# CaptainEven/DenseBox

Hardware: AMD Instinct MI355X
Metric: training patches/sec (240x240) (higher is better)
Workload: dtype f16; 1 GPU; full training step (fwd + fused dense loss w/ hard-negative mining + bwd + grad all-reduce + SGD) of DenseBoxLMLOC on 240x240 patches; net=DenseBoxLMLOC, batch_per_gpu=64, global_batch=64, patch=240x240, parallelism=dp1, half_neg=11, grad_finite=True

## Files before the change

densebox_amd/_lib.py:

```python
import ctypes as C
import os

_HERE = os.path.dirname(os.path.abspath(__file__))
LIB_PATH = os.environ.get('DBX_LIB') or os.path.join(_HERE, 'csrc', 'libdensebox_hip.so')

F16, BF16, F32 = 0, 1, 2
DTYPE_ID = {'f16': F16, 'bf16': BF16, 'f32': F32}
ESIZE = {F16: 2, BF16: 2, F32: 4}

EPI_BIAS, EPI_RELU, EPI_GATE, EPI_DROPMASK, EPI_ACCUM, EPI_F32_NCHW, EPI_DROPHASH = 1, 2, 4, 8, 16, 32, 64
CONV_WFRAG = 128
K_IGEMM, K_DMA, K_BAND, K_C64, K_C8, K_WS, K_P8 = 1, 2, 3, 4, 5, 6, 7


class View(C.Structure):
    _fields_ = [('ptr', C.c_void_p), ('n', C.c_int32), ('h', C.c_int32), ('w', C.c_int32),
                ('pad', C.c_int32), ('ld', C.c_int32), ('c_off', C.c_int32), ('c', C.c_int32)]


class ConvDesc(C.Structure):
    _fields_ = [('dtype', C.c_int32), ('kh', C.c_int32), ('kw', C.c_int32), ('cpad', C.c_int32),
                ('cin_pad', C.c_int32), ('cout_pad', C.c_int32), ('epilogue', C.c_int32), ('drop_seed', C.c_uint32)]


# ... 168 lines not shown
    'dbx_patch_plan_host': (C.c_int, [_I32, _I32, _I32, _VP, _I32, _D, _D, _D, _I32, C.POINTER(PatchGeom)]),
    'dbx_patch_draw': (C.c_int, [_I64, _I64, _I32, _I32, _VP]),
    'dbx_patch_check_tables': (C.c_int, [_VP, _I32, _VP, _I32, _VP, _I32]),
    'dbx_patch_aug_plan': (C.c_int, [C.POINTER(PatchAugIO), C.POINTER(PatchAugCfg), _I32, _VP]),
    'dbx_patch_augment': (C.c_int, [_VP, _VP, _VP, _VP, _I32, _I32, _I32, _VP, _VP]),
    'dbx_patch_aug_params_host': (C.c_int, [C.POINTER(PatchAugCfg), _I64, _I64, _VP, _VP, _I32, _VP, _VP, _VP, _VP, _VP]),
    'dbx_patch_augment_host': (C.c_int, [_VP, _VP, _VP, _I32, _I32, _VP]),
    'dbx_conv_wgrad_scratch_bytes': (_I64, [_I32, _PV, _PV, _I32, _I32]),
    'dbx_conv_wgrad': (C.c_int, [_I32, _PV, _PV, _I32, _I32, _I32, _I32, _I32, _VP, _VP, _VP, _I32, _VP]),
    'dbx_conv_wgrad_slice': (C.c_int, [_I32, _PV, _PV, _I32, _I32, _I32, _I32, _I32, _VP, _I32, _I32, _VP, _VP, _I32, _VP]),
    'dbx_conv_wgrad_pool_dz_ok': (C.c_int, [_I32, _PV, _PV, _I32, _I32]),
    'dbx_conv_wgrad_pool_dz': (C.c_int, [_I32, _PV, _VP, _I32, _PV, _PV, _I32, _I32, _I32, _I32, _I32, _VP, _VP, _VP, _I32, _I32, _VP]),
    'dbx_head2_backward_up_fused': (C.c_int, [_I32, _PV, _PV]),
    'dbx_heads1_wgrad_gen_ok': (C.c_int, [_I32, _PV, _I32]),
    'dbx_heads1_dgrad_gen': (C.c_int, [_I32, _PV, C.POINTER(C.c_void_p), C.POINTER(C.c_int32), _I32, _I32, C.c_uint32, _VP, _PV, _PV, _VP]),
    'dbx_heads1_wgrad_gen': (C.c_int, [_I32, _PV, _PV, C.POINTER(C.c_void_p), C.POINTER(C.c_int32), _I32, _I32, C.c_uint32, _I32, _VP, _I32, _I32,
                             _VP, _VP, _VP]),
    'dbx_conv_wgrad_plan': (C.c_int, [_I32, _PV, _PV, _I32, _I32, C.c_char_p, _I32, C.POINTER(C.c_int32)]),
    'dbx_nchw_to_framed': (C.c_int, [_I32, _VP, _I32, _PV, _VP]),
    'dbx_u8hwc_to_framed': (C.c_int, [_I32, _VP, _PV, C.POINTER(C.c_float), C.POINTER(C.c_float), _VP]),
    'dbx_nchw_to_framed_ch': (C.c_int, [_I32, _VP, _I32, _PV, _I32, _VP]),
    'dbx_nchw_to_framed_slots': (C.c_int, [_I32, _VP, _VP, _I32, _I32, _PV, _VP]),
    'dbx_framed_to_nchw_f32': (C.c_int, [_I32, _PV, _VP, _VP]),
    'dbx_framed_add_ch': (C.c_int, [_I32, _PV, _I32, _I32, _PV, _I32, _VP]),
    'dbx_maxpool2x2': (C.c_int, [_I32, _PV, _PV, _VP]),
    'dbx_maxpool2x2_bwd': (C.c_int, [_I32, _PV, _PV, _PV, _I32, _I32, _VP]),
    'dbx_maxpool_idx_bytes': (C.c_int64, [_I32, _I32, _I32, _I32]),
    'dbx_maxpool2x2_idx': (C.c_int, [_I32, _PV, _PV, _VP, _VP]),
    'dbx_maxpool2x2_bwd_idx': (C.c_int, [_I32, _VP, _PV, _PV, _I32, _I32, _VP]),
    'dbx_upsample_bilinear': (C.c_int, [_I32, _PV, _PV, _VP]),
    'dbx_upsample_bilinear_bwd': (C.c_int, [_I32, _PV, _PV, _PV, _VP]),
    'dbx_loss_scratch_bytes': (C.c_int64, [_I32]),
    'dbx_loss_forward_backward': (C.c_int, [C.POINTER(LossDesc), C.POINTER(LossIO), _VP, _VP]),
    'dbx_count_positives': (C.c_int, [_VP, _VP, _I32, _VP, _VP]),
    'dbx_init_score_map': (C.c_int, [_VP, _VP, _I32, _VP, _VP]),
    'dbx_init_offset_map': (C.c_int, [_VP, _VP, _I32, _I32, _VP, _VP]),
    'dbx_init_lm_heatmap': (C.c_int, [_VP, _VP, _I32, _I32, _VP, _VP]),
# ... 65 lines not shown
```

densebox_amd/csrc/aux_ops.hip:

```cpp
#include "common.hpp"
#include <mutex>

static thread_local char g_err[512] = "";
void dbx_set_error(const char* fmt, ...) {
    va_list ap;
    va_start(ap, fmt);
    vsnprintf(g_err, sizeof(g_err), fmt, ap);
    va_end(ap);
}
extern "C" const char* dbx_last_error(void) { return g_err; }
extern "C" int dbx_version(void) { return DBX_ABI_VERSION; }
extern "C" int dbx_device_arch(int device) {
    hipDeviceProp_t p;
    if (hipGetDeviceProperties(&p, device) != hipSuccess) { dbx_set_error("hipGetDeviceProperties failed"); return DBX_ERR_HIP; }
    int arch = 0;
    const char* s = p.gcnArchName;
    if (s[0] == 'g' && s[1] == 'f' && s[2] == 'x') arch = (int)strtol(s + 3, nullptr, 16) == 0x950 ? 950 : (int)strtol(s + 3, nullptr, 10);
    return arch;
}

template <typename T> struct Vec { static constexpr int N = 16 / sizeof(T); };

template <typename T> __device__ __forceinline__ void load_vec(const T* p, float (&v)[16 / sizeof(T)]) {
    const u32x4 raw = *(const u32x4*)p;
// ... 38 lines not shown
    }
}
template <typename T> static int nchw_to_framed_t(const float* x, int csrc, const dbx_view* y, hipStream_t s) {
    VIEW_VEC_CHECK(T, y, "nchw_to_framed");
    FrameGeo g = make_geo<T>(y);
    const int64_t total = (int64_t)y->n * y->h * y->w * (y->c / Vec<T>::N);
    hipLaunchKernelGGL(nchw_to_framed_kernel<T>, dim3(grid_for(total)), dim3(256), 0, s, x, csrc, g);
    DBX_LAUNCH_CHECK();
    return DBX_OK;
}
extern "C" int dbx_nchw_to_framed(int32_t dtype, const float* x_nchw, int32_t c_src, const dbx_view* y, void* stream) {
    DBX_DISPATCH_DTYPE(dtype, nchw_to_framed_t, x_nchw, c_src, y, (hipStream_t)stream);
}

struct SlotSrc { const float* x[4]; int k[4]; };
template <typename T>
__global__ void nchw_to_framed_slots_kernel(SlotSrc src, int nslots, int slot, FrameGeo y) {
    constexpr int V = Vec<T>::N;
    const int gps = slot / V, cg = nslots * gps;
    const int64_t total = (int64_t)y.n * y.h * y.w * cg;
    for (int64_t i = blockIdx.x * (int64_t)blockDim.x + threadIdx.x; i < total; i += (int64_t)gridDim.x * blockDim.x) {
        const int px = (int)(i % y.w);
        const int g = (int)((i / y.w) % cg);
        const int py = (int)((i / ((int64_t)y.w * cg)) % y.h);
        const int n = (int)(i / ((int64_t)y.w * cg * y.h));
        const int si = g / gps, c0 = (g % gps) * V;
        const float* x = si == 0 ? src.x[0] : si == 1 ? src.x[1] : si == 2 ? src.x[2] : src.x[3];
        const int k = si == 0 ? src.k[0] : si == 1 ? src.k[1] : si == 2 ? src.k[2] : src.k[3];
        float v[V];
#pragma unroll
        for (int j = 0; j < V; ++j) {
            const int c = c0 + j;
            v[j] = (x && c < k) ? x[(((int64_t)n * k + c) * y.h + py) * y.w + px] : 0.f;
        }
        store_vec<T>((T*)y.base + geo_pix(y, n, py, px) + si * slot + c0, v);
    }
}
template <typename T> static int nchw_to_framed_slots_t(const float* const* xs, const int32_t* ks, int nslots, int slot, const dbx_view* y, hipStream_t s) {
    VIEW_VEC_CHECK(T, y, "nchw_to_framed_slots");
    DBX_REQUIRE(nslots >= 1 && nslots <= 4 && slot % Vec<T>::N == 0 && y->c == nslots * slot, "nchw_to_framed_slots: 1..4 slots of a multiple of the vector width, view of nslots * slot channels");
    SlotSrc src;
    for (int i = 0; i < 4; ++i) {
        src.x[i] = i < nslots ? xs[i] : nullptr; src.k[i] = i < nslots ? ks[i] : 0;
        if (i < nslots) DBX_REQUIRE(ks[i] >= 0 && ks[i] <= slot, "nchw_to_framed_slots: k must fit its slot");
    }
    FrameGeo g = make_geo<T>(y);
    const int64_t total = (int64_t)y->n * y->h * y->w * (y->c / Vec<T>::N);
    hipLaunchKernelGGL(nchw_to_framed_slots_kernel<T>, dim3(grid_for(total)), dim3(256), 0, s, src, nslots, slot, g);
    DBX_LAUNCH_CHECK();
    return DBX_OK;
}
extern "C" int dbx_nchw_to_framed_slots(int32_t dtype, const float* const* x_nchw, const int32_t* k, int32_t nslots, int32_t slot, const dbx_view* y,
                                        void* stream) {
    if (!x_nchw || !k || !y) { dbx_set_error("nchw_to_framed_slots: null argument"); return DBX_ERR_ARG; }
    DBX_DISPATCH_DTYPE(dtype, nchw_to_framed_slots_t, x_nchw, k, nslots, slot, y, (hipStream_t)stream);
}

template <typename T>
__global__ void framed_to_nchw_kernel(FrameGeo x, float* __restrict__ y) {
    const int64_t total = (int64_t)x.n * x.c * x.h * x.w;
    for (int64_t i = blockIdx.x * (int64_t)blockDim.x + threadIdx.x; i < total; i += (int64_t)gridDim.x * blockDim.x) {
        const int px = (int)(i % x.w);
        const int py = (int)((i / x.w) % x.h);
        const int c = (int)((i / ((int64_t)x.w * x.h)) % x.c);
        const int n = (int)(i / ((int64_t)x.w * x.h * x.c));
        y[i] = to_f32(((const T*)x.base)[geo_pix(x, n, py, px) + c]);
    }
}
template <typename T> static int framed_to_nchw_t(const dbx_view* x, float* y, hipStream_t s) {
    FrameGeo g = make_geo<T>(x);
// ... 1708 lines not shown
```

densebox_amd/csrc/conv_igemm.hip:

```cpp
#include "common.hpp"
#include <vector>
#include <stdlib.h>
#include <string.h>

struct ConvArgs {
    const char* x;
    const char* w;
    const float* bias;
    char* y;
    const char* gate;
    const unsigned char* dropmask;
    int M, HoWo, Wo;
    int x_hp, x_wp, x_ld, x_org;
    int y_hp, y_wp, y_ld, y_pad;
    int g_hp, g_wp, g_ld, g_pad;
    int kw;
    int ntaps;
    int cpt;
    int ksteps;
    int ktot_bytes;
    int cout_valid;
    int ntile_n;
    int nblocks;
    int epi;
// ... 1841 lines not shown
    DBX_LAUNCH_CHECK();
    return DBX_OK;
}

extern "C" int dbx_pack_weight(int32_t dtype, int32_t mode, const float* w_oihw, int32_t co, int32_t ci, int32_t kh,
                               int32_t kw, void* w_packed, int32_t rows_pad, int32_t cin_pad, int32_t row_off,
                               int32_t k_off, void* stream) {
    DBX_DISPATCH_DTYPE(dtype, pack_weight_t, mode, w_oihw, co, ci, kh, kw, w_packed, rows_pad, cin_pad, row_off, k_off,
                       (hipStream_t)stream);
}

int dbx_internal_heads1_dgrad_gen_f32(const dbx_view* d_out, const float* const* w2, const int32_t* k, int nh, int use_hash, unsigned seed,
                                      const void* w1t_plain, const dbx_view* y, const dbx_view* gate, hipStream_t s);
template <typename T>
static int heads1_dgrad_gen_t(const dbx_view* d_out, const float* const* w2, const int32_t* k, int nh, int use_hash, unsigned seed, const void* w1t_frag,
                              const dbx_view* y, const dbx_view* gate, hipStream_t s) {
    if constexpr (sizeof(T) != 2) return dbx_internal_heads1_dgrad_gen_f32(d_out, w2, k, nh, use_hash, seed, w1t_frag, y, gate, s);
    else {
        DBX_REQUIRE(nh >= 1 && nh <= 4 && d_out->pad == 0 && d_out->n == y->n && d_out->h == y->h && d_out->w == y->w && gate->n == y->n &&
                    gate->h == y->h && gate->w == y->w, "heads1_dgrad_gen: d_out (compact), y and gate are maps of the same pixels");
        DBX_REQUIRE(y->c == 256 && gate->c == 256 && (y->ld * 2) % 16 == 0 && (gate->ld * 2) % 16 == 0 && (y->c_off * 2) % 16 == 0 && (gate->c_off * 2) % 16 == 0 &&
                    ((size_t)y->ptr % 16) == 0 && ((size_t)gate->ptr % 16) == 0 && ((size_t)w1t_frag % 16) == 0, "heads1_dgrad_gen: 256 output channels, 16-byte aligned");
        DBX_REQUIRE(d_out->c % nh == 0 && d_out->c / nh >= 8 && ((size_t)d_out->ptr % 16) == 0 && (d_out->ld * 2) % 16 == 0 && (d_out->c_off * 2) % 16 == 0 &&
                    ((d_out->c / nh) * 2) % 16 == 0, "heads1_dgrad_gen: d_out slots of >= 8 channels, 16-byte aligned");
        const int64_t npix = (int64_t)y->n * y->h * y->w;
        DBX_REQUIRE(npix > 0 && npix < (1 << 24) && npix * d_out->ld * 2 < ((int64_t)1 << 32), "heads1_dgrad_gen: pixel count");
        HGenArgs a;
        a.g.dout = (const char*)d_out->ptr + (size_t)d_out->c_off * 2;
        for (int i = 0; i < 4; ++i) {
            a.g.w2[i] = i < nh ? w2[i] : nullptr; a.g.k[i] = i < nh ? k[i] : 0;
            if (i < nh) DBX_REQUIRE(w2[i] && k[i] >= 1 && k[i] <= 8, "heads1_dgrad_gen: k in 1..8");
        }
        a.g.ld = d_out->ld; a.g.slot = d_out->c / nh; a.g.nh = nh; a.g.H = y->h; a.g.W = y->w; a.g.pad = 0; a.g.seed = seed; a.g.use_hash = use_hash ? 1 : 0;
        a.w1f = (const char*)w1t_frag;
        a.y = (char*)y->ptr + (size_t)y->c_off * 2; a.gate = (const char*)gate->ptr + (size_t)gate->c_off * 2;
        a.y_hp = y->h + 2 * y->pad; a.y_wp = y->w + 2 * y->pad; a.y_ld = y->ld; a.y_pad = y->pad;
        a.g_hp = gate->h + 2 * gate->pad; a.g_wp = gate->w + 2 * gate->pad; a.g_ld = gate->ld; a.g_pad = gate->pad;
        a.npix = (int)npix; a.ntiles = (int)((npix + 255) / 256); a.nhb = 16 * nh;
        return launch_heads1_dgrad_gen<T>(a, s);
    }
}
extern "C" int dbx_heads1_dgrad_gen(int32_t dtype, const dbx_view* d_out, const float* const* w2, const int32_t* k, int32_t nh, int32_t use_hash,
                                    uint32_t drop_seed, const void* w1t_frag, const dbx_view* y, const dbx_view* gate, void* stream) {
    if (!d_out || !w2 || !k || !w1t_frag || !y || !gate) { dbx_set_error("heads1_dgrad_gen: null argument"); return DBX_ERR_ARG; }
    DBX_DISPATCH_DTYPE(dtype, heads1_dgrad_gen_t, d_out, w2, k, nh, use_hash, (unsigned)drop_seed, w1t_frag, y, gate, (hipStream_t)stream);
}
```

densebox_amd/csrc/heads_gen.hpp:

```cpp
#pragma once

#ifndef HG_ABL
#define HG_ABL 0
#endif
namespace hgen {
constexpr int HB_BYTES = 16384, NST = 4, W2T_BYTES = 2048 * 16 + 64, LUT_BYTES = 256 * 16;
constexpr int SMEM = NST * HB_BYTES + W2T_BYTES + LUT_BYTES;
}
struct HGenArgs {
    GenHid g;
    const char* w1f;
    char* y; const char* gate;
    int y_hp, y_wp, y_ld, y_pad, g_hp, g_wp, g_ld, g_pad;
    int npix, ntiles, nhb;
};

template <typename T>
__global__ __launch_bounds__(256, 1) void heads1_dgrad_gen_kernel(const HGenArgs a) {
    static_assert(sizeof(T) == 2, "16-bit compute types");
    using namespace hgen;
    extern __shared__ __attribute__((aligned(16))) char smem[];
    char* const w2t = smem + NST * HB_BYTES;
    char* const lut = w2t + W2T_BYTES;
    const int tid = threadIdx.x, lane = tid & 63, l31 = lane & 31, lh = lane >> 5;
    const int wave = __builtin_amdgcn_readfirstlane(tid >> 6);
    const int nhb = a.nhb;
    {
        const float sc = a.g.use_hash ? 2.f : 1.f;
        for (int c = tid; c < 32 * nhb; c += 256) {
            const int hd = c >> 9, cl = c & 511;
// ... 30 lines not shown
        unsigned keep;
        asm volatile("s_mov_b32 %0, m0\n\ts_mov_b32 m0, %3\n\ts_nop 0\n\tglobal_load_lds_dwordx4 %1, %2\n\ts_mov_b32 m0, %0"
                     : "=&s"(keep) : "v"(voff), "s"(src), "s"(dst) : "memory");
    };
    const unsigned vlane = (unsigned)lane * 16u;
    int wb_next = 0, st_next = 0;
    auto issue = [&]() {
        const char* src = a.w1f + (size_t)wb_next * HB_BYTES + wave * 4096;
        const unsigned dst = lds0 + st_next * HB_BYTES + wave * 4096;
#pragma unroll
        for (int q = 0; q < 4; ++q) glds(src + q * 1024, vlane, dst + q * 1024);
        if (++wb_next == nhb) wb_next = 0;
        st_next = (st_next + 1) & 3;
    };

    const int stride = gridDim.x;
    int tile = blockIdx.x;
    if (tile >= a.ntiles) return;
    int m[2]; unsigned hm[2]; bool ok[2];
    auto set_tile = [&](int t) {
#pragma unroll
        for (int pf = 0; pf < 2; ++pf) {
            const int mm = t * 256 + wave * 64 + pf * 32 + l31;
            ok[pf] = mm < a.npix;
            m[pf] = ok[pf] ? mm : a.npix - 1;
            hm[pf] = (unsigned)m[pf] * 0x9E3779B1u;
        }
    };
    u32x4 dnx[2];
    auto dfetch = [&](int t, int hd) {
// ... 46 lines not shown
                for (int p = 0; p < 4; ++p)
                    o[p] = __builtin_bit_cast(unsigned, __builtin_convertvector((f32x2v){dd[pf][8 * t + 2 * p], dd[pf][8 * t + 2 * p + 1]}, t2v)) & mk[pf][t][p];
                bfr[buf][pf][t] = o;
            }
    };
    auto gen = [&](int buf, int hb, const u32x4& wa) { gen_mma(wa); gen_masks(hb); gen_pack(buf); };

    f32x16 acc[2][8];
#pragma unroll
    for (int pf = 0; pf < 2; ++pf)
#pragma unroll
        for (int cf = 0; cf < 8; ++cf)
#pragma unroll
            for (int r = 0; r < 16; ++r) acc[pf][cf][r] = 0.f;

    issue(); issue(); issue();
    set_tile(tile);
    dfetch(tile, 0);
    asm volatile("s_waitcnt vmcnt(0)" : "+v"(dnx[0]), "+v"(dnx[1]) :: "memory");
    __syncthreads();
    dswap();
    gen(0, 0, gen_w(0));

    int st = 0;
    for (;;) {
        for (int hb = 0; hb < nhb; hb += 2) {
#pragma unroll
            for (int par = 0; par < 2; ++par) {
                const int h = hb + par;
                asm volatile("s_waitcnt vmcnt(8)" : "+v"(dnx[0]), "+v"(dnx[1]) :: "memory");
                __builtin_amdgcn_s_barrier();
                const char* S = smem + st * HB_BYTES + lane * 16;
                const bool last = h + 1 == nhb;
                const u32x4 wa = gen_w(last ? 0 : h + 1);
                u32x4 wf0[8], wf1[8];
#pragma unroll
                for (int cf = 0; cf < 8; ++cf) wf0[cf] = *(const u32x4*)(S + cf * 1024);
                __builtin_amdgcn_sched_barrier(0);
                if (!(HG_ABL & 8)) issue();
                if ((h & 15) == 12) {
                    const bool wrap = h + 4 >= nhb;
                    dfetch(wrap ? tile + stride : tile, wrap ? 0 : (h + 4) >> 4);
                }
                if ((h & 15) == 15) {
                    if (last) set_tile(tile + stride);
                    dswap();
                }
                if (!(HG_ABL & 1)) { gen_mma(wa); gen_masks(last ? 0 : h + 1); }
                __builtin_amdgcn_sched_barrier(0);
#pragma unroll
                for (int cf = 0; cf < 8; ++cf) {
                    wf1[cf] = *(const u32x4*)(S + (8 + cf) * 1024);
                    if (HG_ABL & 4) continue;
                    Mma32<T>::run(wf0[cf], bfr[par][0][0], acc[0][cf]);
                    Mma32<T>::run(wf0[cf], bfr[par][1][0], acc[1][cf]);
                    __builtin_amdgcn_sched_group_barrier(0x100, 1, 0);
                    __builtin_amdgcn_sched_group_barrier(0x008, 2, 0);
                }
                __builtin_amdgcn_sched_barrier(0);
                if (!(HG_ABL & 1)) gen_pack(par ^ 1);
#pragma unroll
                for (int cf = 0; cf < 8; ++cf) {
                    if (HG_ABL & 4) continue;
                    Mma32<T>::run(wf1[cf], bfr[par][0][1], acc[0][cf]);
                    Mma32<T>::run(wf1[cf], bfr[par][1][1], acc[1][cf]);
                    __builtin_amdgcn_sched_group_barrier(0x008, 2, 0);
                    __builtin_amdgcn_sched_group_barrier(0x002, 4, 0);
                }
                st = (st + 1) & 3;
            }
        }
        __builtin_amdgcn_sched_barrier(0);
        if (!(HG_ABL & 2)) {
            T* ypix[2];
            bool okp[2];
            u32x4 gt[2][8][2];
#pragma unroll
            for (int pf = 0; pf < 2; ++pf) {
                const int mm = tile * 256 + wave * 64 + pf * 32 + l31;
                okp[pf] = mm < a.npix;
                const int mc = okp[pf] ? mm : 0;
                const int hw = a.g.H * a.g.W;
                const int n = mc / hw, rem = mc - n * hw, oy = rem / a.g.W, ox = rem - oy * a.g.W;
                ypix[pf] = (T*)a.y + (size_t)((n * a.y_hp + oy + a.y_pad) * a.y_wp + ox + a.y_pad) * (size_t)a.y_ld + 8 * lh;
                const T* gpix = (const T*)a.gate + (size_t)((n * a.g_hp + oy + a.g_pad) * a.g_wp + ox + a.g_pad) * (size_t)a.g_ld + 8 * lh;
#pragma unroll
                for (int cf = 0; cf < 8; ++cf)
// ... 13 lines not shown
                            T p4[4] = {from_f32<T>(acc[pf][cf][4 * j]), from_f32<T>(acc[pf][cf][4 * j + 1]), from_f32<T>(acc[pf][cf][4 * j + 2]),
                                       from_f32<T>(acc[pf][cf][4 * j + 3])};
                            pk[jj] = *(const u32x2*)p4;
                        }
                        const auto r0 = __builtin_amdgcn_permlane32_swap(pk[0].x, pk[1].x, false, false);
                        const auto r1 = __builtin_amdgcn_permlane32_swap(pk[0].y, pk[1].y, false, false);
                        const u32x4 o = gate_packed16((u32x4){r0[0], r1[0], r0[1], r1[1]}, gt[pf][cf][jp]);
                        if (okp[pf]) *(u32x4*)(ypix[pf] + cf * 32 + 16 * jp) = o;
                    }
#pragma unroll
                    for (int r = 0; r < 16; ++r) acc[pf][cf][r] = 0.f;
                }
            }
        }
        __builtin_amdgcn_sched_barrier(0);
        tile += stride;
        if (tile >= a.ntiles) break;
    }
    asm volatile("s_waitcnt vmcnt(0)" ::: "memory");
}

template <typename T>
static int launch_heads1_dgrad_gen(const HGenArgs& a, hipStream_t s) {
    static DbxDevOnce attr_once; int attr_dev = 0;
    if (attr_once.pending(&attr_dev)) {
        DBX_HIP(hipFuncSetAttribute((const void*)heads1_dgrad_gen_kernel<T>, hipFuncAttributeMaxDynamicSharedMemorySize, hgen::SMEM));
        attr_once.mark(attr_dev);
    }
    int ncu = 0, dev = 0;
    if (hipGetDevice(&dev) != hipSuccess || hipDeviceGetAttribute(&ncu, hipDeviceAttributeMultiprocessorCount, dev) != hipSuccess || ncu <= 0) ncu = 256;
// ... 6 lines not shown
```

densebox_amd/engine.py:

```python
import ctypes as C
import os
import weakref

import torch

from . import _lib
from ._lib import View, ConvDesc, check, ptr, stream_ptr

_BACKBONE = [('conv1_1_1', 3, 64), ('conv1_2_1', 64, 64), ('conv2_1_1', 64, 128), ('conv2_2_1', 128, 128),
             ('conv3_1_1', 128, 256), ('conv3_2_1', 256, 256), ('conv3_4_1', 256, 256),
             ('conv4_1_1', 256, 512), ('conv4_2_1', 512, 512), ('conv4_3_1', 512, 512), ('conv4_4_1', 512, 512)]

_HEADS = {
    'DenseBox': [('det', 1), ('loc', 4)],
    'DenseBoxLM': [('det', 1), ('loc', 4), ('landmark', 4)],
    'DenseBoxLMLOC': [('det', 1), ('loc', 4), ('landmark', 4), ('lmloc', 8)],
}


_FWD_IO = {'conv1_1_1': ('x0', 'a11'), 'conv1_2_1': ('a11', 'a12'), 'conv2_1_1': ('p1', 'a21'), 'conv2_2_1': ('a21', 'a22'),
           'conv3_1_1': ('p2', 'a31'), 'conv3_2_1': ('a31', 'a32'), 'conv3_4_1': ('a32', 'c34'), 'conv4_1_1': ('p3', 'a41'),
           'conv4_2_1': ('a41', 'a42'), 'conv4_3_1': ('a42', 'a43'), 'conv4_4_1': ('a43', 'a44')}
_BWD_IO = {'conv4_4_1': ('d_a44', 'd_a43'), 'conv4_3_1': ('d_a43', 'd_a42'), 'conv4_2_1': ('d_a42', 'd_a41'),
           'conv4_1_1': ('d_a41', 'd_p3'), 'conv3_4_1': ('d_c34', 'd_a32'), 'conv3_2_1': ('d_a32', 'd_a31'),
# ... 1001 lines not shown
            dgrad('conv6_3_det', d_rfo, B['d_rf_u'].view(), 1, 1, 0, 64, P.crf)
            check(L.dbx_upsample_bilinear_bwd(dt, C.byref(B['d_rf_u'].view()), C.byref(B['d_rf_2'].view()), None, s))
            conv_bwd('conv6_2_det', B['d_rf_2'].view(), B['rf_1'].view(), 5, 5, 0, 64, 64)
            dgrad('conv6_2_det', B['d_rf_2'].view(), B['d_rf_1'].view(), 5, 5, 4, 64, 64)
            conv_bwd('conv6_1_det', B['d_rf_1'].view(), B['rf_p'].view(), 3, 3, 0, 64, 5)
            dgrad('conv6_1_det', B['d_rf_1'].view(), B['d_rf_p'].view(), 3, 3, 2, 64, 64)
            check(L.dbx_maxpool2x2_bwd(dt, C.byref(B['rf_in'].view()), C.byref(B['d_rf_p'].view()),
                                       C.byref(B['d_rf_in'].view()), 0, 0, s))

        slot = {}
        srcs = []
        for i, (stem, k) in enumerate(heads):
            slot[stem] = B['d_out'].view(P.crf * i, P.crf)
            src = override.get(stem)
            srcs.append(src if src is not None else gout(stem, k))
        if override or kind == 'DenseBox':
            check(L.dbx_nchw_to_framed_slots(dt, (C.c_void_p * nh)(*[t.data_ptr() for t in srcs]), (C.c_int32 * nh)(*[k for _, k in heads]), nh, P.crf,
                                             C.byref(B['d_out'].view()), s))
        else:
            for (stem, k), t in zip(heads, srcs):
                check(L.dbx_nchw_to_framed(dt, ptr(t), k, C.byref(slot[stem]), s))
        if kind != 'DenseBox' and not override:
            check(L.dbx_framed_add_ch(dt, C.byref(B['d_rf_in'].view()), 0, 4, C.byref(slot['landmark']), 0, s))
            check(L.dbx_framed_add_ch(dt, C.byref(B['d_rf_in'].view()), 4, 1, C.byref(slot['det']), 0, s))

        hv = B['hid'].view()
        need = L.dbx_head2_wgrad_scratch_bytes(nh, hv.n * hv.h)
        if getattr(self, '_h2_scratch', None) is None or self._h2_scratch.numel() < need:
            self._h2_scratch = torch.empty(int(need), dtype=torch.uint8, device=dev)
        dw2 = [new_grad('conv5_2_%s.weight' % st) for st, _ in heads]
        db2 = [new_grad('conv5_2_%s.bias' % st) for st, _ in heads]
        prof = self.profile
        if prof is not None:
# ... 66 lines not shown
            if sink is not None:
                sink.ready(w1n + b1n)
        on_side(run_h1)
        for i, (stem, _) in enumerate(heads):
            G['conv5_1_%s.weight' % stem] = dw1[512 * i:512 * (i + 1)]
            G['conv5_1_%s.bias' % stem] = db1[512 * i:512 * (i + 1)]
        row_bytes = 512 * nh * _lib.ESIZE[dt]
        if lin:
            fa, fc = self._frag_heads(P, dt, 'ba'), self._frag_heads(P, dt, 'bc')
            self._conv(dt, B['d_g44'].view(), B['d_a44'].view(), self._w_heads1_bwd_part(dt, 'a', frag=fa), None, 1, 1, 0, 512 * nh, 512,
                       _lib.EPI_GATE | (_lib.CONV_WFRAG if fa else 0), gate=B['a44'].view())
            if gen:
                if prof is not None:
                    ev0, ev1 = torch.cuda.Event(enable_timing=True), torch.cuda.Event(enable_timing=True)
                    ev0.record()
                check(L.dbx_heads1_dgrad_gen(dt, C.byref(B['d_out'].view()), w2p, ks, nh, hash_on, hash_seed,
                                             ptr(self._w_heads1_bwd_part(dt, 'c', frag=dt != _lib.F32)), C.byref(B['d_c34'].view()), C.byref(c34), s))
                if prof is not None:
                    ev1.record()
                    prof.append({'kernel': 'heads1_dgrad_gen_kernel<%s>' % ('f16', 'bf16', 'f32')[dt],
                                 'flops': 2.0 * hv.n * hv.h * hv.w * 512 * nh * (256 + 8), 'start': ev0, 'end': ev1})
            else:
                if fc and getattr(P, 'heads_gen', False):
                    fc = self.conv_plan(dt, dhid_v, B['d_c34'].view(), 1, 1, 0, 512 * nh, 256, _lib.EPI_GATE)[2]
                self._conv(dt, dhid_v, B['d_c34'].view(), self._w_heads1_bwd_part(dt, 'c', frag=fc), None, 1, 1, 0, 512 * nh, 256,
                           _lib.EPI_GATE | (_lib.CONV_WFRAG if fc else 0), gate=c34)
        elif dt != _lib.F32:
            bfrag = self._frag_heads(P, dt, 'b')
            w1t = self._w_heads1_bwd(dt, frag=bfrag)
            d = ConvDesc(dt, 1, 1, 0, 512 * nh, 768, _lib.CONV_WFRAG if bfrag else 0, 0)
            prof = self.profile
            if prof is not None:
# ... 89 lines not shown
```

include/densebox_hip.h:

```cpp
#ifndef DENSEBOX_HIP_H
#define DENSEBOX_HIP_H

#include <stdint.h>

#ifdef __cplusplus
extern "C" {
#endif

enum dbx_status {
    DBX_OK = 0,
    DBX_ERR_ARG = -1,
    DBX_ERR_HIP = -2,
    DBX_ERR_DTYPE = -3
};

enum dbx_dtype { DBX_F16 = 0, DBX_BF16 = 1, DBX_F32 = 2 };

const char* dbx_last_error(void);
#define DBX_ABI_VERSION 13
int dbx_version(void);
int dbx_device_arch(int device);

typedef struct dbx_view {
    void*   ptr;
// ... 76 lines not shown
                       uint32_t drop_seed, float* const* dw, float* const* db, void* scratch, void* stream);
int dbx_head2_backward_up(int32_t dtype, const dbx_view* d_out, const dbx_view* hid, const float* const* w2, const int32_t* k,
                          int32_t nh, const dbx_view* d_hid, const uint8_t* dropmask, int32_t dropmask_ld, int32_t use_hash,
                          uint32_t drop_seed, float* const* dw, float* const* db, void* scratch, const dbx_view* d_g44, void* stream);
int dbx_conv_wgrad_pool_dz_ok(int32_t dtype, const dbx_view* dz, const dbx_view* x, int32_t kh, int32_t kw);
int dbx_conv_wgrad_pool_dz(int32_t dtype, const dbx_view* dy, const void* idx, int32_t idx_channels, const dbx_view* dz, const dbx_view* x,
                           int32_t kh, int32_t kw, int32_t cpad, int32_t co, int32_t ci, float* dw_oihw, float* db, void* scratch,
                           int32_t accumulate, int32_t write_dz, void* stream);
int dbx_head2_backward_up_fused(int32_t dtype, const dbx_view* hid, const dbx_view* d_g44);
int dbx_heads1_wgrad_gen_ok(int32_t dtype, const dbx_view* x, int32_t nh);
int dbx_heads1_wgrad_gen(int32_t dtype, const dbx_view* d_out, const dbx_view* x, const float* const* w2, const int32_t* k, int32_t nh,
                         int32_t use_hash, uint32_t drop_seed, int32_t ci, float* dw_oihw, int32_t dw_ci_total, int32_t dw_ci_off,
                         float* db, void* scratch, void* stream);
int dbx_heads1_dgrad_gen(int32_t dtype, const dbx_view* d_out, const float* const* w2, const int32_t* k, int32_t nh, int32_t use_hash,
                         uint32_t drop_seed, const void* w1t_frag, const dbx_view* y, const dbx_view* gate, void* stream);

int dbx_fold_heads(const float* w2, const float* b2, const float* w1, const float* b1, int32_t k, float* w_out,
                   float* b_out, void* stream);
int dbx_fold_refine(const float* w1, const float* b1, const float* w2, const float* b2, const float* w3, const float* b3,
                    int32_t ci, int32_t cm, float* w_out, float* b_out, float* v_out, void* stream);
int dbx_refine_eval(const float* landmark_nchw, const float* score_nchw, int32_t n, int32_t h, int32_t w, const float* w_fold,
                    const float* b_fold, float* out_small, void* stream);
int dbx_upsample_bilinear_nchw_f32(const float* x, int32_t planes, int32_t hi, int32_t wi, float* y, int32_t ho, int32_t wo,
                                   void* stream);
int64_t dbx_refine_backward_scratch_bytes(int32_t n, int32_t h, int32_t w);
int dbx_refine_backward(const float* d_refine, const float* landmark, const float* score, int32_t n, int32_t h, int32_t w,
                        const float* w1, const float* b1, const float* w2, const float* b2, const float* w3, const float* b3,
                        int32_t cm, const float* w_fold, const float* v_fold, const float* g_landmark, const float* g_score, float* out_landmark,
                        float* out_score, float* dw1, float* db1, float* dw2, float* db2, float* dw3, float* db3, void* scratch,
                        void* stream);
// ... 7 lines not shown
int dbx_conv_wgrad_plan(int32_t dtype, const dbx_view* dz, const dbx_view* x, int32_t kh, int32_t kw, char* name, int32_t name_len,
                        int32_t* splits);

int64_t dbx_conv_dgrad_wgrad1_scratch_bytes(void);
int dbx_conv_dgrad_wgrad1_fusable(const dbx_conv_desc* d, const dbx_view* dz, const dbx_view* gate, const dbx_view* x0);
int dbx_conv_dgrad_wgrad1(const dbx_conv_desc* d, const dbx_view* dz, const void* w_packed, const dbx_view* gate, const dbx_view* x0,
                          int32_t ci, float* dw_oihw, float* db, void* scratch, int32_t accumulate, void* stream);

int dbx_nchw_to_framed(int32_t dtype, const float* x_nchw, int32_t c_src, const dbx_view* y, void* stream);
int dbx_u8hwc_to_framed(int32_t dtype, const uint8_t* x_nhwc, const dbx_view* y, const float* mean3, const float* std3,
                        void* stream);
int dbx_nchw_to_framed_ch(int32_t dtype, const float* x_nchw, int32_t c_src, const dbx_view* y, int32_t c_dst_off,
                          void* stream);
int dbx_nchw_to_framed_slots(int32_t dtype, const float* const* x_nchw, const int32_t* k, int32_t nslots, int32_t slot,
                             const dbx_view* y, void* stream);
int dbx_framed_to_nchw_f32(int32_t dtype, const dbx_view* x, float* y_nchw, void* stream);
int dbx_framed_add_ch(int32_t dtype, const dbx_view* src, int32_t c_src_off, int32_t n_ch, const dbx_view* dst,
                      int32_t c_dst_off, void* stream);
int dbx_maxpool2x2(int32_t dtype, const dbx_view* x, const dbx_view* y, void* stream);
int dbx_maxpool2x2_bwd(int32_t dtype, const dbx_view* x, const dbx_view* dy, const dbx_view* dx,
                       int32_t accumulate, int32_t relu_gate, void* stream);
int64_t dbx_maxpool_idx_bytes(int32_t n, int32_t h, int32_t w, int32_t c);
int dbx_maxpool2x2_idx(int32_t dtype, const dbx_view* x, const dbx_view* y, void* idx, void* stream);
int dbx_maxpool2x2_bwd_idx(int32_t dtype, const void* idx, const dbx_view* dy, const dbx_view* dx,
                           int32_t accumulate, int32_t relu_gate, void* stream);
int dbx_upsample_bilinear(int32_t dtype, const dbx_view* x, const dbx_view* y, void* stream);
int dbx_upsample_bilinear_bwd(int32_t dtype, const dbx_view* dy, const dbx_view* dx, const dbx_view* gate, void* stream);

typedef struct dbx_loss_desc {
    int32_t kind;
// ... 271 lines not shown
```

Baseline: 7592 patches/s.

## Skip zero-gradient head blocks in heads1 dgrad using per-row nonzero flags

The framing kernel that packs head output gradients now records, per head and image row, an epoch-stamped flag whenever any packed value is nonzero. The heads1 dgrad kernel reads these flags for each 256-pixel tile and, for heads whose rows are all zero, runs a variant of the pipeline that skips the LDS weight loads and MFMA work while keeping the issue and prefetch cadence. With hard-negative mining many loss gradients are exactly zero, so this targets wasted matrix work. It adds flag writes, scalar flag loads per tile, and code-size growth from the duplicated block.

```diff
diff --git a/densebox_amd/_lib.py b/densebox_amd/_lib.py
--- a/densebox_amd/_lib.py
+++ b/densebox_amd/_lib.py
@@ -206,6 +206,8 @@
     'dbx_head2_backward_up_fused': (C.c_int, [_I32, _PV, _PV]),
     'dbx_heads1_wgrad_gen_ok': (C.c_int, [_I32, _PV, _I32]),
     'dbx_heads1_dgrad_gen': (C.c_int, [_I32, _PV, C.POINTER(C.c_void_p), C.POINTER(C.c_int32), _I32, _I32, C.c_uint32, _VP, _PV, _PV, _VP]),
+    'dbx_heads1_dgrad_gen_flags': (C.c_int, [_I32, _PV, C.POINTER(C.c_void_p), C.POINTER(C.c_int32), _I32, _I32, C.c_uint32, _VP, _PV, _PV, _VP,
+                                             C.c_uint32, _VP]),
     'dbx_heads1_wgrad_gen': (C.c_int, [_I32, _PV, _PV, C.POINTER(C.c_void_p), C.POINTER(C.c_int32), _I32, _I32, C.c_uint32, _I32, _VP, _I32, _I32,
                              _VP, _VP, _VP]),
     'dbx_conv_wgrad_plan': (C.c_int, [_I32, _PV, _PV, _I32, _I32, C.c_char_p, _I32, C.POINTER(C.c_int32)]),
@@ -213,6 +215,7 @@
     'dbx_u8hwc_to_framed': (C.c_int, [_I32, _VP, _PV, C.POINTER(C.c_float), C.POINTER(C.c_float), _VP]),
     'dbx_nchw_to_framed_ch': (C.c_int, [_I32, _VP, _I32, _PV, _I32, _VP]),
     'dbx_nchw_to_framed_slots': (C.c_int, [_I32, _VP, _VP, _I32, _I32, _PV, _VP]),
+    'dbx_nchw_to_framed_slots_flags': (C.c_int, [_I32, _VP, _VP, _I32, _I32, _PV, _VP, C.c_uint32, _VP]),
     'dbx_framed_to_nchw_f32': (C.c_int, [_I32, _PV, _VP, _VP]),
     'dbx_framed_add_ch': (C.c_int, [_I32, _PV, _I32, _I32, _PV, _I32, _VP]),
     'dbx_maxpool2x2': (C.c_int, [_I32, _PV, _PV, _VP]),
diff --git a/densebox_amd/csrc/aux_ops.hip b/densebox_amd/csrc/aux_ops.hip
--- a/densebox_amd/csrc/aux_ops.hip
+++ b/densebox_amd/csrc/aux_ops.hip
@@ -76,8 +76,8 @@
 }
 
 struct SlotSrc { const float* x[4]; int k[4]; };
-template <typename T>
-__global__ void nchw_to_framed_slots_kernel(SlotSrc src, int nslots, int slot, FrameGeo y) {
+template <typename T, bool FL>
+__global__ void nchw_to_framed_slots_kernel(SlotSrc src, int nslots, int slot, FrameGeo y, unsigned* __restrict__ row_flags, unsigned epoch) {
     constexpr int V = Vec<T>::N;
     const int gps = slot / V, cg = nslots * gps;
     const int64_t total = (int64_t)y.n * y.h * y.w * cg;
@@ -96,9 +96,16 @@
             v[j] = (x && c < k) ? x[(((int64_t)n * k + c) * y.h + py) * y.w + px] : 0.f;
         }
         store_vec<T>((T*)y.base + geo_pix(y, n, py, px) + si * slot + c0, v);
-    }
-}
-template <typename T> static int nchw_to_framed_slots_t(const float* const* xs, const int32_t* ks, int nslots, int slot, const dbx_view* y, hipStream_t s) {
+        if constexpr (FL) {
+            bool nz = false;
+#pragma unroll
+            for (int j = 0; j < V; ++j) nz = nz || to_f32(from_f32<T>(v[j])) != 0.f;
+            if (nz) row_flags[((size_t)si * y.n + n) * y.h + py] = epoch;
+        }
+    }
+}
+template <typename T> static int nchw_to_framed_slots_t(const float* const* xs, const int32_t* ks, int nslots, int slot, const dbx_view* y, hipStream_t s,
+                                                        unsigned* row_flags = nullptr, unsigned epoch = 0) {
     VIEW_VEC_CHECK(T, y, "nchw_to_framed_slots");
     DBX_REQUIRE(nslots >= 1 && nslots <= 4 && slot % Vec<T>::N == 0 && y->c == nslots * slot, "nchw_to_framed_slots: 1..4 slots of a multiple of the vector width, view of nslots * slot channels");
     SlotSrc src;
@@ -108,7 +115,8 @@
     }
     FrameGeo g = make_geo<T>(y);
     const int64_t total = (int64_t)y->n * y->h * y->w * (y->c / Vec<T>::N);
-    hipLaunchKernelGGL(nchw_to_framed_slots_kernel<T>, dim3(grid_for(total)), dim3(256), 0, s, src, nslots, slot, g);
+    if (row_flags) hipLaunchKernelGGL((nchw_to_framed_slots_kernel<T, true>), dim3(grid_for(total)), dim3(256), 0, s, src, nslots, slot, g, row_flags, epoch);
+    else hipLaunchKernelGGL((nchw_to_framed_slots_kernel<T, false>), dim3(grid_for(total)), dim3(256), 0, s, src, nslots, slot, g, nullptr, 0u);
     DBX_LAUNCH_CHECK();
     return DBX_OK;
 }
@@ -116,6 +124,12 @@
                                         void* stream) {
     if (!x_nchw || !k || !y) { dbx_set_error("nchw_to_framed_slots: null argument"); return DBX_ERR_ARG; }
     DBX_DISPATCH_DTYPE(dtype, nchw_to_framed_slots_t, x_nchw, k, nslots, slot, y, (hipStream_t)stream);
+}
+extern "C" int dbx_nchw_to_framed_slots_flags(int32_t dtype, const float* const* x_nchw, const int32_t* k, int32_t nslots, int32_t slot,
+                                              const dbx_view* y, uint32_t* row_flags, uint32_t epoch, void* stream) {
+    if (!x_nchw || !k || !y || !row_flags) { dbx_set_error("nchw_to_framed_slots_flags: null argument"); return DBX_ERR_ARG; }
+    if (epoch == 0 || ((size_t)row_flags & 3)) { dbx_set_error("nchw_to_framed_slots_flags: epoch must not be 0, flags 4-byte aligned"); return DBX_ERR_ARG; }
+    DBX_DISPATCH_DTYPE(dtype, nchw_to_framed_slots_t, x_nchw, k, nslots, slot, y, (hipStream_t)stream, (unsigned*)row_flags, (unsigned)epoch);
 }
 
 template <typename T>
diff --git a/densebox_amd/csrc/conv_igemm.hip b/densebox_amd/csrc/conv_igemm.hip
--- a/densebox_amd/csrc/conv_igemm.hip
+++ b/densebox_amd/csrc/conv_igemm.hip
@@ -1879,7 +1879,7 @@
                                       const void* w1t_plain, const dbx_view* y, const dbx_view* gate, hipStream_t s);
 template <typename T>
 static int heads1_dgrad_gen_t(const dbx_view* d_out, const float* const* w2, const int32_t* k, int nh, int use_hash, unsigned seed, const void* w1t_frag,
-                              const dbx_view* y, const dbx_view* gate, hipStream_t s) {
+                              const dbx_view* y, const dbx_view* gate, hipStream_t s, const uint32_t* row_flags = nullptr, uint32_t epoch = 0) {
     if constexpr (sizeof(T) != 2) return dbx_internal_heads1_dgrad_gen_f32(d_out, w2, k, nh, use_hash, seed, w1t_frag, y, gate, s);
     else {
         DBX_REQUIRE(nh >= 1 && nh <= 4 && d_out->pad == 0 && d_out->n == y->n && d_out->h == y->h && d_out->w == y->w && gate->n == y->n &&
@@ -1902,6 +1902,9 @@
         a.y_hp = y->h + 2 * y->pad; a.y_wp = y->w + 2 * y->pad; a.y_ld = y->ld; a.y_pad = y->pad;
         a.g_hp = gate->h + 2 * gate->pad; a.g_wp = gate->w + 2 * gate->pad; a.g_ld = gate->ld; a.g_pad = gate->pad;
         a.npix = (int)npix; a.ntiles = (int)((npix + 255) / 256); a.nhb = 16 * nh;
+        a.use_flags = row_flags ? 1 : 0;
+        a.flags = row_flags ? (const unsigned*)row_flags : (const unsigned*)w1t_frag;
+        a.epoch = epoch; a.rows = row_flags ? y->n * y->h : 0;
         return launch_heads1_dgrad_gen<T>(a, s);
     }
 }
@@ -1910,3 +1913,10 @@
     if (!d_out || !w2 || !k || !w1t_frag || !y || !gate) { dbx_set_error("heads1_dgrad_gen: null argument"); return DBX_ERR_ARG; }
     DBX_DISPATCH_DTYPE(dtype, heads1_dgrad_gen_t, d_out, w2, k, nh, use_hash, (unsigned)drop_seed, w1t_frag, y, gate, (hipStream_t)stream);
 }
+extern "C" int dbx_heads1_dgrad_gen_flags(int32_t dtype, const dbx_view* d_out, const float* const* w2, const int32_t* k, int32_t nh, int32_t use_hash,
+                                          uint32_t drop_seed, const void* w1t_frag, const dbx_view* y, const dbx_view* gate, const uint32_t* row_flags,
+                                          uint32_t epoch, void* stream) {
+    if (!d_out || !w2 || !k || !w1t_frag || !y || !gate) { dbx_set_error("heads1_dgrad_gen: null argument"); return DBX_ERR_ARG; }
+    if (row_flags && (epoch == 0 || ((size_t)row_flags & 3))) { dbx_set_error("heads1_dgrad_gen: epoch must not be 0, flags 4-byte aligned"); return DBX_ERR_ARG; }
+    DBX_DISPATCH_DTYPE(dtype, heads1_dgrad_gen_t, d_out, w2, k, nh, use_hash, (unsigned)drop_seed, w1t_frag, y, gate, (hipStream_t)stream, row_flags, epoch);
+}
diff --git a/densebox_amd/csrc/heads_gen.hpp b/densebox_amd/csrc/heads_gen.hpp
--- a/densebox_amd/csrc/heads_gen.hpp
+++ b/densebox_amd/csrc/heads_gen.hpp
@@ -13,7 +13,10 @@
     char* y; const char* gate;
     int y_hp, y_wp, y_ld, y_pad, g_hp, g_wp, g_ld, g_pad;
     int npix, ntiles, nhb;
+    const unsigned* flags;
+    unsigned epoch; int rows, use_flags;
 };
+template <int I> struct HGenIC { static constexpr int v = I; };
 
 template <typename T>
 __global__ __launch_bounds__(256, 1) void heads1_dgrad_gen_kernel(const HGenArgs a) {
@@ -74,6 +77,11 @@
         st_next = (st_next + 1) & 3;
     };
 
+    auto advance = [&]() {
+        if (++wb_next == nhb) wb_next = 0;
+        st_next = (st_next + 1) & 3;
+    };
+
     const int stride = gridDim.x;
     int tile = blockIdx.x;
     if (tile >= a.ntiles) return;
@@ -150,8 +158,40 @@
 #pragma unroll
             for (int r = 0; r < 16; ++r) acc[pf][cf][r] = 0.f;
 
+    constexpr int ZR = 6;
+    typedef const unsigned __attribute__((address_space(4))) cu32;
+    cu32* const fl = (cu32*)(uintptr_t)a.flags;
+    unsigned fw[4][ZR];
+    bool fwide = false;
+    auto zfetch = [&](int t) {
+        const int tt = t < a.ntiles ? t : a.ntiles - 1;
+        const int p0 = tt * 256, p1 = p0 + 255 < a.npix ? p0 + 255 : a.npix - 1;
+        const int r0 = a.use_flags ? p0 / a.g.W : 0, r1 = a.use_flags ? p1 / a.g.W : 0;
+        fwide = r1 - r0 >= ZR;
+#pragma unroll
+        for (int hd = 0; hd < 4; ++hd)
+#pragma unroll
+            for (int j = 0; j < ZR; ++j) {
+                const int r = r0 + j < r1 ? r0 + j : r1, hh = 16 * hd < nhb ? hd : 0;
+                fw[hd][j] = fl[hh * a.rows + r];
+            }
+    };
+    auto zmask = [&]() -> unsigned {
+        unsigned z = 0;
+#pragma unroll
+        for (int hd = 0; hd < 4; ++hd) {
+            bool any = false;
+#pragma unroll
+            for (int j = 0; j < ZR; ++j) any = any || fw[hd][j] == a.epoch;
+            if (!any) z |= 1u << hd;
+        }
+        return (a.use_flags && !fwide) ? z : 0u;
+    };
+
     issue(); issue(); issue();
     set_tile(tile);
+    zfetch(tile);
+    unsigned zt = zmask();
     dfetch(tile, 0);
     asm volatile("s_waitcnt vmcnt(0)" : "+v"(dnx[0]), "+v"(dnx[1]) :: "memory");
     __syncthreads();
@@ -159,54 +199,73 @@
     gen(0, 0, gen_w(0));
 
     int st = 0;
+    auto block = [&](auto full_c, auto par_c, const int h) __attribute__((always_inline)) {
+        constexpr bool FULL = decltype(full_c)::v != 0;
+        constexpr int par = decltype(par_c)::v;
+        asm volatile("s_waitcnt vmcnt(8)" : "+v"(dnx[0]), "+v"(dnx[1]) :: "memory");
+        __builtin_amdgcn_s_barrier();
+        const char* S = smem + st * HB_BYTES + lane * 16;
+        const bool last = h + 1 == nhb;
+        const u32x4 wa = gen_w(last ? 0 : h + 1);
+        u32x4 wf0[8], wf1[8];
+        if constexpr (FULL) {
+#pragma unroll
+            for (int cf = 0; cf < 8; ++cf) wf0[cf] = *(const u32x4*)(S + cf * 1024);
+        }
+        __builtin_amdgcn_sched_barrier(0);
+        if constexpr (FULL) { if (!(HG_ABL & 8)) issue(); }
+        else { if ((h & 15) >= 13) issue(); else advance(); }
+        if ((h & 15) == 12) {
+            const bool wrap = h + 4 >= nhb;
+            dfetch(wrap ? tile + stride : tile, wrap ? 0 : (h + 4) >> 4);
+        }
+        if ((h & 15) == 15) {
+            if (last) set_tile(tile + stride);
+            dswap();
+        }
+        if (!(HG_ABL & 1)) { gen_mma(wa); gen_masks(last ? 0 : h + 1); }
+        __builtin_amdgcn_sched_barrier(0);
+        if constexpr (FULL) {
+#pragma unroll
+            for (int cf = 0; cf < 8; ++cf) {
+                wf1[cf] = *(const u32x4*)(S + (8 + cf) * 1024);
+                if (HG_ABL & 4) continue;
+                Mma32<T>::run(wf0[cf], bfr[par][0][0], acc[0][cf]);
+                Mma32<T>::run(wf0[cf], bfr[par][1][0], acc[1][cf]);
+                __builtin_amdgcn_sched_group_barrier(0x100, 1, 0);
+                __builtin_amdgcn_sched_group_barrier(0x008, 2, 0);
+            }
+            __builtin_amdgcn_sched_barrier(0);
+        }
+        if (!(HG_ABL & 1)) gen_pack(par ^ 1);
+        if constexpr (FULL) {
+#pragma unroll
+            for (int cf = 0; cf < 8; ++cf) {
+                if (HG_ABL & 4) continue;
+                Mma32<T>::run(wf1[cf], bfr[par][0][1], acc[0][cf]);
+                Mma32<T>::run(wf1[cf], bfr[par][1][1], acc[1][cf]);
+                __builtin_amdgcn_sched_group_barrier(0x008, 2, 0);
+                __builtin_amdgcn_sched_group_barrier(0x002, 4, 0);
+            }
+        }
+        st = (st + 1) & 3;
+    };
     for (;;) {
-        for (int hb = 0; hb < nhb; hb += 2) {
-#pragma unroll
-            for (int par = 0; par < 2; ++par) {
-                const int h = hb + par;
-                asm volatile("s_waitcnt vmcnt(8)" : "+v"(dnx[0]), "+v"(dnx[1]) :: "memory");
-                __builtin_amdgcn_s_barrier();
-                const char* S = smem + st * HB_BYTES + lane * 16;
-                const bool last = h + 1 == nhb;
-                const u32x4 wa = gen_w(last ? 0 : h + 1);
-                u32x4 wf0[8], wf1[8];
-#pragma unroll
-                for (int cf = 0; cf < 8; ++cf) wf0[cf] = *(const u32x4*)(S + cf * 1024);
-                __builtin_amdgcn_sched_barrier(0);
-                if (!(HG_ABL & 8)) issue();
-                if ((h & 15) == 12) {
-                    const bool wrap = h + 4 >= nhb;
-                    dfetch(wrap ? tile + stride : tile, wrap ? 0 : (h + 4) >> 4);
+        for (int hd = 0; hd < nhb; hd += 16) {
+            if ((zt >> (hd >> 4)) & 1u) {
+                for (int hb = hd; hb < hd + 16; hb += 2) {
+                    block(HGenIC<0>{}, HGenIC<0>{}, hb);
+                    block(HGenIC<0>{}, HGenIC<1>{}, hb + 1);
                 }
-                if ((h & 15) == 15) {
-                    if (last) set_tile(tile + stride);
-                    dswap();
+            } else {
+                for (int hb = hd; hb < hd + 16; hb += 2) {
+                    block(HGenIC<1>{}, HGenIC<0>{}, hb);
+                    block(HGenIC<1>{}, HGenIC<1>{}, hb + 1);
                 }
-                if (!(HG_ABL & 1)) { gen_mma(wa); gen_masks(last ? 0 : h + 1); }
-                __builtin_amdgcn_sched_barrier(0);
-#pragma unroll
-                for (int cf = 0; cf < 8; ++cf) {
-                    wf1[cf] = *(const u32x4*)(S + (8 + cf) * 1024);
-                    if (HG_ABL & 4) continue;
-                    Mma32<T>::run(wf0[cf], bfr[par][0][0], acc[0][cf]);
-                    Mma32<T>::run(wf0[cf], bfr[par][1][0], acc[1][cf]);
-                    __builtin_amdgcn_sched_group_barrier(0x100, 1, 0);
-                    __builtin_amdgcn_sched_group_barrier(0x008, 2, 0);
-                }
-                __builtin_amdgcn_sched_barrier(0);
-                if (!(HG_ABL & 1)) gen_pack(par ^ 1);
-#pragma unroll
-                for (int cf = 0; cf < 8; ++cf) {
-                    if (HG_ABL & 4) continue;
-                    Mma32<T>::run(wf1[cf], bfr[par][0][1], acc[0][cf]);
-                    Mma32<T>::run(wf1[cf], bfr[par][1][1], acc[1][cf]);
-                    __builtin_amdgcn_sched_group_barrier(0x008, 2, 0);
-                    __builtin_amdgcn_sched_group_barrier(0x002, 4, 0);
-                }
-                st = (st + 1) & 3;
             }
         }
         __builtin_amdgcn_sched_barrier(0);
+        zfetch(tile + stride);
         if (!(HG_ABL & 2)) {
             T* ypix[2];
             bool okp[2];
@@ -250,6 +309,7 @@
             }
         }
         __builtin_amdgcn_sched_barrier(0);
+        zt = zmask();
         tile += stride;
         if (tile >= a.ntiles) break;
     }
diff --git a/densebox_amd/engine.py b/densebox_amd/engine.py
--- a/densebox_amd/engine.py
+++ b/densebox_amd/engine.py
@@ -1039,9 +1039,19 @@
             slot[stem] = B['d_out'].view(P.crf * i, P.crf)
             src = override.get(stem)
             srcs.append(src if src is not None else gout(stem, k))
+        rf_p, rf_epoch = None, 0
         if override or kind == 'DenseBox':
-            check(L.dbx_nchw_to_framed_slots(dt, (C.c_void_p * nh)(*[t.data_ptr() for t in srcs]), (C.c_int32 * nh)(*[k for _, k in heads]), nh, P.crf,
-                                             C.byref(B['d_out'].view()), s))
+            xs_p, ks_p = (C.c_void_p * nh)(*[t.data_ptr() for t in srcs]), (C.c_int32 * nh)(*[k for _, k in heads])
+            if dt != _lib.F32 and os.environ.get('DBX_HEADS_ROWSKIP', '1') != '0' and not torch.cuda.is_current_stream_capturing():
+                rf = getattr(P, 'row_flags', None)
+                if rf is None or getattr(P, 'row_epoch', 0) >= 0xfffffff0:
+                    rf = P.row_flags = torch.zeros(nh * n * h4, dtype=torch.int32, device=dev)
+                    P.row_epoch = 0
+                P.row_epoch += 1
+                rf_p, rf_epoch = C.c_void_p(rf.data_ptr()), P.row_epoch
+                check(L.dbx_nchw_to_framed_slots_flags(dt, xs_p, ks_p, nh, P.crf, C.byref(B['d_out'].view()), rf_p, rf_epoch, s))
+            else:
+                check(L.dbx_nchw_to_framed_slots(dt, xs_p, ks_p, nh, P.crf, C.byref(B['d_out'].view()), s))
         else:
             for (stem, k), t in zip(heads, srcs):
                 check(L.dbx_nchw_to_framed(dt, ptr(t), k, C.byref(slot[stem]), s))
@@ -1138,8 +1148,9 @@
                 if prof is not None:
                     ev0, ev1 = torch.cuda.Event(enable_timing=True), torch.cuda.Event(enable_timing=True)
                     ev0.record()
-                check(L.dbx_heads1_dgrad_gen(dt, C.byref(B['d_out'].view()), w2p, ks, nh, hash_on, hash_seed,
-                                             ptr(self._w_heads1_bwd_part(dt, 'c', frag=dt != _lib.F32)), C.byref(B['d_c34'].view()), C.byref(c34), s))
+                check(L.dbx_heads1_dgrad_gen_flags(dt, C.byref(B['d_out'].view()), w2p, ks, nh, hash_on, hash_seed,
+                                                   ptr(self._w_heads1_bwd_part(dt, 'c', frag=dt != _lib.F32)), C.byref(B['d_c34'].view()), C.byref(c34),
+                                                   rf_p, rf_epoch, s))
                 if prof is not None:
                     ev1.record()
                     prof.append({'kernel': 'heads1_dgrad_gen_kernel<%s>' % ('f16', 'bf16', 'f32')[dt],
diff --git a/include/densebox_hip.h b/include/densebox_hip.h
--- a/include/densebox_hip.h
+++ b/include/densebox_hip.h
@@ -114,6 +114,9 @@
                          float* db, void* scratch, void* stream);
 int dbx_heads1_dgrad_gen(int32_t dtype, const dbx_view* d_out, const float* const* w2, const int32_t* k, int32_t nh, int32_t use_hash,
                          uint32_t drop_seed, const void* w1t_frag, const dbx_view* y, const dbx_view* gate, void* stream);
+int dbx_heads1_dgrad_gen_flags(int32_t dtype, const dbx_view* d_out, const float* const* w2, const int32_t* k, int32_t nh, int32_t use_hash,
+                               uint32_t drop_seed, const void* w1t_frag, const dbx_view* y, const dbx_view* gate, const uint32_t* row_flags,
+                               uint32_t epoch, void* stream);
 
 int dbx_fold_heads(const float* w2, const float* b2, const float* w1, const float* b1, int32_t k, float* w_out,
                    float* b_out, void* stream);
@@ -151,6 +154,8 @@
                           void* stream);
 int dbx_nchw_to_framed_slots(int32_t dtype, const float* const* x_nchw, const int32_t* k, int32_t nslots, int32_t slot,
                              const dbx_view* y, void* stream);
+int dbx_nchw_to_framed_slots_flags(int32_t dtype, const float* const* x_nchw, const int32_t* k, int32_t nslots, int32_t slot,
+                                   const dbx_view* y, uint32_t* row_flags, uint32_t epoch, void* stream);
 int dbx_framed_to_nchw_f32(int32_t dtype, const dbx_view* x, float* y_nchw, void* stream);
 int dbx_framed_add_ch(int32_t dtype, const dbx_view* src, int32_t c_src_off, int32_t n_ch, const dbx_view* dst,
                       int32_t c_dst_off, void* stream);
```

After: 7621 patches/s, median of 6. About the same (+0.4%).
